# fundamentalvision/BEVFormer

Measured on NVIDIA H100. Metric: BEV queries/sec (bevformer_base 200x200x256, 6 cams) fwd+bwd, higher is better.
Workload: dtype bf16

## Files before the change

### bevformer_b200/_lib.py

```python
from __future__ import annotations

import ctypes
import os
import threading

from . import build as _build

_lock = threading.Lock()
_lib = None

c_void_p, c_int, c_int64 = ctypes.c_void_p, ctypes.c_int, ctypes.c_int64

SIGNATURES = {
    "bevf_version": (c_int, []),
    "bevf_last_error": (ctypes.c_char_p, []),
    "bevf_launch_count": (c_int64, []),
    "bevf_msda_forward": (c_int, [c_void_p, c_int, c_void_p, c_void_p, c_void_p, c_void_p,
                                  c_void_p, c_int] + [c_int] * 7 + [c_void_p]),
    "bevf_msda_backward": (c_int, [c_void_p, c_int, c_void_p, c_void_p, c_void_p, c_void_p,
                                   c_void_p, c_int, c_void_p, c_void_p, c_void_p] + [c_int] * 7
                           + [c_void_p]),
    "bevf_msda_rows_forward": (c_int, [c_void_p, c_int, c_void_p, c_void_p, c_void_p, c_void_p,
                                       c_void_p, c_int, c_void_p] + [c_int] * 7 + [c_void_p]),
    "bevf_msda_rows_backward": (c_int, [c_void_p, c_int, c_void_p, c_void_p, c_void_p, c_void_p,
                                        c_void_p, c_int, c_void_p, c_void_p, c_void_p, c_void_p]
                                + [c_int] * 7 + [c_void_p]),
    "bevf_msda_rows_backward_ordered": (c_int, [c_void_p, c_int, c_void_p, c_void_p, c_void_p, c_void_p,
                                                c_void_p, c_int, c_void_p, c_void_p, c_void_p, c_void_p,
                                                c_void_p] + [c_int] * 7 + [c_void_p]),
    "bevf_msda_set_backward_mode": (c_int, [c_int]),
    "bevf_abs_max": (c_int, [c_void_p, c_int, c_int64, c_void_p, c_void_p]),
    "bevf_msda_rows_backward_f16acc": (c_int, [c_void_p, c_int, c_void_p, c_void_p, c_void_p, c_void_p, c_void_p, c_int,
                                               c_void_p, c_void_p, c_void_p, c_void_p, c_void_p, c_void_p] + [c_int] * 7
                                       + [c_void_p]),
    "bevf_gv16_unscale": (c_int, [c_void_p, c_void_p, c_void_p, c_int64, c_void_p]),
    "bevf_msda_rows_backward_mixed": (c_int, [c_void_p, c_int, c_void_p, c_void_p, c_void_p, c_void_p, c_void_p, c_void_p,
                                              c_int, c_void_p, c_void_p, c_void_p, c_int, c_void_p, c_void_p, c_void_p,
                                              c_void_p] + [c_int] * 7 + [c_void_p]),
    "bevf_msda_rows_backward_mixed_dense": (c_int, [c_void_p, c_int, c_void_p, c_void_p, c_void_p, c_void_p, c_void_p,
                                                    c_void_p, c_int, c_void_p, c_void_p, c_void_p, c_int, c_int,
                                                    c_void_p, c_void_p, c_void_p, c_void_p] + [c_int] * 7 + [c_void_p]),
    "bevf_gv_merge": (c_int, [c_void_p, c_void_p, c_void_p, c_void_p, c_int, c_int, c_int, c_int, c_void_p]),
    "bevf_msda_fx_frac_bits": (c_int, [c_int64, c_int, c_int]),
    "bevf_msda_backward_fx": (c_int, [c_void_p, c_int, c_void_p, c_void_p, c_void_p, c_void_p, c_void_p, c_int,
                                      c_void_p, c_void_p, c_int, c_void_p, c_void_p] + [c_int] * 7 + [c_void_p]),
    "bevf_msda_rows_backward_fx": (c_int, [c_void_p, c_int, c_void_p, c_void_p, c_void_p, c_void_p, c_void_p, c_int,
                                           c_void_p, c_void_p, c_int, c_void_p, c_void_p, c_void_p] + [c_int] * 7
                                   + [c_void_p]),
    "bevf_msda_fx_convert": (c_int, [c_void_p, c_void_p, c_int, c_void_p, c_int, c_int, c_int64, c_void_p]),
    "bevf_msda_rows_backward_dense": (c_int, [c_void_p, c_int, c_void_p, c_void_p, c_void_p, c_void_p, c_void_p,
                                              c_void_p, c_int, c_void_p, c_void_p, c_void_p, c_void_p, c_void_p]
                                      + [c_int] * 7 + [c_void_p]),
    "bevf_msda_set_dense_backward": (c_int, [c_int]),
    "bevf_msda_get_dense_backward": (c_int, []),
    "bevf_msda_dense_plan": (c_int, [c_void_p, c_int, c_int, c_int, c_void_p, c_int, c_void_p]),
    "bevf_sca_plan_workspace_ints": (c_int64, [c_int, c_int]),
    "bevf_sca_plan_build": (c_int, [c_void_p] * 10 + [c_int] * 5 + [c_void_p]),
    "bevf_sca_prep_forward": (c_int, [c_void_p] * 7 + [c_int] * 8 + [c_void_p]),
    "bevf_sca_prep_backward": (c_int, [c_void_p] * 6 + [c_int] * 8 + [c_void_p]),
    "bevf_sca_rows_forward_fused": (c_int, [c_void_p, c_int] + [c_void_p] * 9 + [c_int, c_void_p, c_int, c_void_p]
                                    + [c_int] * 12 + [c_void_p]),
    "bevf_sca_rows_backward_fused": (c_int, [c_void_p, c_int] + [c_void_p] * 7 + [c_int] + [c_void_p] * 5
                                     + [c_int, c_void_p, c_void_p, c_void_p, c_int, c_int] + [c_void_p] * 5
                                     + [c_int] * 12 + [c_void_p]),
    "bevf_sca_prep_backward_multi": (c_int, [c_void_p] * 6 + [c_int] * 8 + [c_void_p]),
    "bevf_tsa_prep_forward": (c_int, [c_void_p] * 5 + [c_int] * 6 + [c_void_p]),
    "bevf_tsa_prep_backward": (c_int, [c_void_p] * 5 + [c_int] * 7 + [c_void_p]),
    "bevf_query_prep_forward": (c_int, [c_void_p] * 5 + [c_int] * 7 + [c_void_p]),
    "bevf_query_prep_backward": (c_int, [c_void_p] * 5 + [c_int] * 8 + [c_void_p]),
    "bevf_refine_points": (c_int, [c_void_p, c_int64, c_void_p, c_void_p, c_void_p, c_int, c_int64, c_void_p]),
    "bevf_layernorm_forward": (c_int, [c_void_p] * 4 + [c_int] + [c_void_p] * 5
                               + [c_int64, c_int, ctypes.c_float, ctypes.c_float, ctypes.c_uint64, c_void_p,
                                  c_int, c_void_p]),
    "bevf_layernorm_backward": (c_int, [c_void_p] * 3 + [c_int] + [c_void_p] * 4 + [c_int64]
                                + [c_void_p] * 4
                                + [c_int64, c_int, ctypes.c_float, ctypes.c_uint64, c_void_p, c_int,
                                   c_void_p]),
    "bevf_layernorm_backward_workspace_bytes": (c_int64, [c_int64, c_int]),
    "bevf_layernorm_backward_det": (c_int, [c_void_p] * 3 + [c_int] + [c_void_p] * 4 + [c_int64]
                                    + [c_void_p] * 5 + [c_int64]
                                    + [c_int64, c_int, ctypes.c_float, ctypes.c_uint64, c_void_p, c_int,
                                       c_void_p]),
    "bevf_sca_combine_forward": (c_int, [c_void_p] * 4 + [c_int] * 6 + [c_void_p]),
    "bevf_sca_combine_backward": (c_int, [c_void_p] * 4 + [c_int] * 5 + [c_void_p]),
    "bevf_linear_forward": (c_int, [c_void_p] * 3 + [c_int] + [c_void_p] * 2
                            + [c_int, c_int64, c_int, c_int, c_int, c_void_p]),
    "bevf_flatten_feats": (c_int, [c_void_p] * 4 + [c_int] * 7 + [c_void_p]),
    "bevf_linear_dgrad": (c_int, [c_void_p] * 3 + [c_int64, c_int, c_int, c_void_p]),
    "bevf_linear_dgrad_acc": (c_int, [c_void_p] * 4 + [c_int64, c_int, c_int, c_void_p]),
    "bevf_linear_wgrad": (c_int, [c_void_p] * 4 + [c_int64, c_int, c_int, c_void_p]),
    "bevf_linear_wgrad_workspace_bytes": (c_int64, [c_int64, c_int, c_int]),
    "bevf_linear_wgrad_out": (c_int, [c_void_p] * 4 + [c_int, c_void_p, c_int64, c_int64, c_int, c_int,
                                                      c_void_p]),
    "bevf_sum_tensors": (c_int, [c_void_p, c_int, c_void_p, c_int64, c_int, c_void_p]),
    "bevf_linear_wgrad_into": (c_int, [c_void_p] * 5 + [c_int64, c_int64, c_int, c_int, c_void_p]),
    "bevf_linear_forward_dt": (c_int, [c_void_p] * 3 + [c_int] + [c_void_p] * 2
                               + [c_int, c_int64, c_int, c_int, c_int, c_int, c_void_p]),
    "bevf_linear_dgrad_dt": (c_int, [c_void_p] * 3 + [c_int64, c_int, c_int, c_int, c_void_p]),
    "bevf_linear_dgrad_acc_dt": (c_int, [c_void_p] * 4 + [c_int64, c_int, c_int, c_int, c_void_p]),
    "bevf_linear_wgrad_dt": (c_int, [c_void_p] * 4 + [c_int64, c_int, c_int, c_int, c_void_p]),
    "bevf_linear_wgrad_out_dt": (c_int, [c_void_p] * 4 + [c_int, c_void_p, c_int64, c_int64, c_int, c_int, c_int,
                                                         c_void_p]),
    "bevf_linear_wgrad_into_dt": (c_int, [c_void_p] * 5 + [c_int64, c_int64, c_int, c_int, c_int, c_void_p]),
    "bevf_colsum": (c_int, [c_void_p, c_void_p, c_int64, c_int, c_int, c_void_p]),
    "bevf_colsum_workspace_bytes": (c_int64, [c_int64, c_int]),
    "bevf_colsum_det": (c_int, [c_void_p, c_void_p, c_void_p, c_int64, c_int64, c_int, c_int, c_void_p]),
    "bevf_dropout_inplace": (c_int, [c_void_p, c_int64, ctypes.c_float, ctypes.c_uint64, c_void_p, c_int,
                                     c_void_p]),
# ... 75 lines not shown
```

### bevformer_b200/csrc/msda.cu

```cuda
#include <cuda_fp16.h>

#include <cstdlib>
#include <cstring>
#include <mutex>
#include <type_traits>

#include "msda_common.cuh"

namespace bevf {

template <typename T, typename TO, bool kFused = false>
__global__ void __launch_bounds__(kThreads)
msda_fwd_d32(const T *__restrict__ value, const int64_t *__restrict__ level_hw,
             const int64_t *__restrict__ level_start, const float *__restrict__ loc,
             const float *__restrict__ attn, TO *__restrict__ out,
             const int *__restrict__ row_map, int S, int M, int Q, int L, int P, int magic,
             int iters, long long rows, const __grid_constant__ ScaFuse fz = ScaFuse{}) {
    constexpr int VEC = Vec<T>::N, LANES = 32 / VEC, G = 32 / LANES;
    static_assert(!kFused || LANES == 4, "the fused prep needs 4 lanes per row (16-bit value rows)");
    constexpr bool kHalf = std::is_same<T, bf16>::value;
    __shared__ __align__(16) float s_fa[kFused ? kThreads / 32 * G : 1][kFuseLP];
    __shared__ LevelTab tab;
    load_level_tab(level_hw, level_start, L, M * 32, tab);

// ... 514 lines not shown
    return 0;
}

template <typename T, typename TO>
static int launch_fwd(const char *who, const void *value, const int64_t *hw, const int64_t *ls,
                      const float *loc, const float *attn, void *out, const int *row_map, int S,
                      int M, int D, int Q, int L, int P, long long rows, cudaStream_t st,
                      const ScaFuse *fz = nullptr) {
    if (D == 32) {
        const unsigned grid = grid_d32(rows, Vec<T>::N);
        if (fz) {
            if constexpr (std::is_same<T, bf16>::value && std::is_same<TO, bf16>::value)
                msda_fwd_d32<T, TO, true><<<grid, kThreads, 0, st>>>((const T *)value, hw, ls, nullptr, nullptr, (TO *)out,
                                                                     row_map, S, M, Q, L, P, (65536 + P - 1) / P, 1,
                                                                     rows, *fz);
            else
                return fail("%s: the fused prep needs bf16 value and output", who);
        } else {
            msda_fwd_d32<T, TO><<<grid, kThreads, 0, st>>>((const T *)value, hw, ls, loc, attn, (TO *)out,
                                                           row_map, S, M, Q, L, P, (65536 + P - 1) / P, 1,
                                                           rows);
        }
    } else if (fz) {
        return fail("%s: the fused prep needs head_dim 32", who);
    } else {
        const unsigned grid = (unsigned)((rows + kThreads / 32 - 1) / (kThreads / 32));
        msda_fwd_generic<T, TO><<<grid, kThreads, 0, st>>>((const T *)value, hw, ls, loc, attn,
                                                           (TO *)out, row_map, S, M, D, Q, L, P, rows);
    }
    return check_launch(who);
}

static std::atomic<int> g_bwd_mode{-1};
static int bwd_split_enabled() {
    int v = g_bwd_mode.load(std::memory_order_relaxed);
    if (v < 0) {
        const char *e = getenv("BEVF_MSDA_BWD");
        v = (e && e[0] == 's') ? 1 : 0;
        g_bwd_mode.store(v, std::memory_order_relaxed);
    }
    return v;
}
static unsigned splat_direct_mask() {
    static long v = -1;
    if (v < 0) {
        const char *e = getenv("BEVF_SPLAT_DIRECT");
        v = e ? strtol(e, nullptr, 0) : 0;
    }
    return (unsigned)v;
}

int dense_coarse_backward(const char *who, const int64_t *hw_dev, const int64_t *ls_dev, const int32_t *hw_host,
                          const float *loc, const float *attn, const void *grad_out, float *grad_value,
                          const int32_t *map_range, int NB, int S, int M, int L, int P, cudaStream_t st,
                          unsigned *handled, HostLevels *host_levels, int first_level, unsigned need_mask,
                          int gv_S, int gv_base, int loc_level0);

static cudaStream_t g_side_stream = nullptr;
constexpr int kSideEvents = 64;
static cudaEvent_t g_side_events[kSideEvents];
static std::atomic<unsigned> g_side_ev_next{0};

template <typename TG, int kM>
static int launch_splat_km(const char *who, const float *loc, const float *attn, const void *go, float *gv,
                           const int *row_map, const int *order, const int64_t *hw, const int64_t *ls,
                           int S, int M, int Q, int L, int P, long long pairs, unsigned level_mask,
                           cudaStream_t st) {
    static bool attr_done = false;
    if (!attr_done) {
        if (cudaFuncSetAttribute(msda_bwd_splat_d32<TG, kM>, cudaFuncAttributeMaxDynamicSharedMemorySize,
                                 (int)splat_smem_bytes(kSplatMaxHeads, sizeof(TG))) != cudaSuccess) {
            cudaGetLastError();
            return fail("%s: cannot reserve shared memory for the splat kernel", who);
        }
        attr_done = true;
    }
    const unsigned grid = (unsigned)((pairs + kSplatG - 1) / kSplatG);
    msda_bwd_splat_d32<TG, kM><<<grid, 32 * M, splat_smem_bytes(M, sizeof(TG)), st>>>(
        loc, attn, (const TG *)go, gv, row_map, order, hw, ls, S, M, Q, L, P, pairs, splat_direct_mask(),
        level_mask);
    return check_launch(who);
}

template <typename TG>
static int launch_splat(const char *who, const float *loc, const float *attn, const void *go, float *gv,
                        const int *row_map, const int *order, const int64_t *hw, const int64_t *ls,
                        int S, int M, int Q, int L, int P, long long pairs, unsigned level_mask,
                        cudaStream_t st) {
    if constexpr (std::is_same<TG, __half>::value) {
        return fail("%s: the splat kernel takes fp32 or bf16 grad_out", who);
    } else {
        if (M == 8)
            return launch_splat_km<TG, 8>(who, loc, attn, go, gv, row_map, order, hw, ls, S, M, Q, L, P, pairs,
                                          level_mask, st);
        return launch_splat_km<TG, 0>(who, loc, attn, go, gv, row_map, order, hw, ls, S, M, Q, L, P, pairs,
                                      level_mask, st);
    }
}

struct MixedGv {
    const unsigned *amax = nullptr;
    __half *gv16 = nullptr;
    unsigned mask = 0;
    int side_start = 0, S_side = 0;
};

struct FxGv {
    const unsigned *bounds = nullptr;
    int frac_bits = 0;
// ... 246 lines not shown
    cudaStream_t s = nullptr;
    if (cudaStreamCreateWithFlags(&s, cudaStreamNonBlocking) != cudaSuccess) {
        cudaGetLastError();
        return fail("%s: cannot create the second stream", who);
    }
    for (int i = 0; i < kSideEvents; ++i) cudaEventCreateWithFlags(&g_side_events[i], cudaEventDisableTiming);
    g_side_stream = s;
    return 0;
}

extern "C" int bevf_msda_set_dense_backward(int mode) {
    if (mode < -1 || mode > 2)
        return fail("%s: mode must be -1 (library default), 0 (off), 1 (same stream) or 2 (second stream)",
                    "bevf_msda_set_dense_backward");
    if (mode == 2)
        if (int e = ensure_side_stream("bevf_msda_set_dense_backward")) return e;
    g_dense_mode.store(mode, std::memory_order_relaxed);
    return 0;
}

extern "C" int bevf_msda_get_dense_backward(void) { return mixed_dense_mode(); }

extern "C" int bevf_msda_rows_backward_dense(const void *value, int value_dtype, const int64_t *level_hw,
                                             const int64_t *level_start, const int32_t *level_hw_host,
                                             const float *loc, const float *attn, const void *grad_out,
                                             int grad_out_dtype, float *grad_value, float *grad_loc,
                                             float *grad_attn, const int32_t *row_map, const int32_t *map_range,
                                             int B, int S, int M, int D, int R, int L, int P, void *stream) {
    const char *who = "bevf_msda_rows_backward_dense";
    if (!row_map && R > 0) return fail("%s: row_map is null", who);
    if (int e = check_dims(who, B, S, M, D, R, L, P)) return e;
    if (R == 0) return 0;
    if (!level_hw_host || !map_range || !level_hw || !level_start || !loc || !attn || !grad_out || !grad_value)
        return fail("%s: null pointer argument", who);
    cudaStream_t st = (cudaStream_t)stream;
    unsigned handled = 0;
    HostLevels hl;
    memset(&hl, 0, sizeof(hl));
    const int mode = dense_setting() < 0 ? 0 : dense_setting();
    cudaEvent_t join = nullptr;
    if (value_dtype == BEVF_DTYPE_F16 || grad_out_dtype == BEVF_DTYPE_F16)
        return fail("%s: fp32 or bf16 only (fp16 runs on bevf_msda_rows_backward)", who);
    if (mode != 0 && D == 32 && grad_out_dtype == BEVF_DTYPE_BF16 && aligned16(loc) && aligned16(attn) &&
        aligned16(grad_out) && aligned16(grad_value)) {
        cudaStream_t ds = st;
        if (mode == 2 && g_side_stream) {
            cudaEvent_t fork = g_side_events[g_side_ev_next.fetch_add(1) % kSideEvents];
            join = g_side_events[g_side_ev_next.fetch_add(1) % kSideEvents];
            cudaEventRecord(fork, st);
            cudaStreamWaitEvent(g_side_stream, fork, 0);
            ds = g_side_stream;
        }
        const int e = dense_coarse_backward(who, level_hw, level_start, level_hw_host, loc, attn, grad_out, grad_value,
                                            map_range, B, S, M, L, P, ds, &handled, &hl, 0, 0u, S, 0, 0);
        if (join) cudaEventRecord(join, g_side_stream);
        if (e) {
            if (join) cudaStreamWaitEvent(st, join, 0);
            return e;
        }
    }
    const int e = msda_backward_impl(who, value, value_dtype, level_hw, level_start, loc, attn, grad_out,
                                     grad_out_dtype, grad_value, grad_loc, grad_attn, row_map, nullptr, B, S, M, D,
                                     R, L, P, stream, handled, &hl);
    if (join) cudaStreamWaitEvent(st, join, 0);
    return e;
}

extern "C" int bevf_msda_rows_backward_f16acc(const void *value, int value_dtype, const int64_t *level_hw,
                                              const int64_t *level_start, const float *loc, const float *attn,
                                              const void *grad_out, int grad_out_dtype, void *grad_value_f16,
                                              const uint32_t *amax_bits, float *grad_loc, float *grad_attn,
                                              const int32_t *row_map, const int32_t *group_order, int B, int S,
                                              int M, int D, int R, int L, int P, void *stream) {
    const char *who = "bevf_msda_rows_backward_f16acc";
    if (!row_map && R > 0) return fail("%s: row_map is null", who);
    if (!grad_value_f16 || !amax_bits) return fail("%s: null pointer argument", who);
    MixedGv mx;
    mx.amax = amax_bits;
    return msda_backward_impl(who, value, value_dtype, level_hw, level_start, loc, attn, grad_out, grad_out_dtype,
                              reinterpret_cast<float *>(grad_value_f16), grad_loc, grad_attn, row_map, group_order, B, S,
                              M, D, R, L, P, stream, 0u, nullptr, true, &mx);
}

static int rows_backward_mixed_impl(const char *who, const void *value, int value_dtype, const int64_t *level_hw,
                                    const int64_t *level_start, const int32_t *level_hw_host, const float *loc,
                                    const float *attn, const void *grad_out, int grad_out_dtype,
                                    void *grad_value_fine_f16, float *grad_value_side, const uint32_t *amax_bits,
                                    int num_f16_levels, int first_dense_level, float *grad_loc, float *grad_attn,
                                    const int32_t *row_map, const int32_t *group_order, const int32_t *map_range,
                                    int B, int S, int M, int D, int R, int L, int P, void *stream,
                                    const ScaFuse *fz = nullptr) {
    if (!row_map && R > 0) return fail("%s: row_map is null", who);
    if (!level_hw_host || !grad_value_fine_f16 || !grad_value_side || !amax_bits)
        return fail("%s: null pointer argument", who);
    if (L <= 1 || L > kMaxLevels || num_f16_levels < 1 || num_f16_levels >= L)
        return fail("%s: num_f16_levels must be in [1, L - 1]", who);
    if (map_range && (first_dense_level < num_f16_levels || first_dense_level >= L))
        return fail("%s: first_dense_level must be in [num_f16_levels, L - 1]", who);
    if (value_dtype != BEVF_DTYPE_BF16 || D != 32) return fail("%s: needs a bf16 value tensor and head_dim 32", who);
    if (!aligned16(grad_value_fine_f16) || !aligned16(grad_value_side))
        return fail("%s: device pointers must be 16-byte aligned", who);
    HostLevels hl;
    memset(&hl, 0, sizeof(hl));
    long long start = 0;
    for (int l = 0; l < L; ++l) {
        const int h = level_hw_host[2 * l], w = level_hw_host[2 * l + 1];
        if (h <= 0 || w <= 0 || h >= 32768 || w >= 32768) return fail("%s: bad host level shape", who);
        hl.h[l] = h; hl.w[l] = w; hl.start[l] = (int)start;
        start += (long long)h * w;
    }
    if (start != S) return fail("%s: host level shapes do not add up to S (%lld vs %lld)", who, start, S);
    MixedGv mx;
    mx.amax = amax_bits;
    mx.gv16 = reinterpret_cast<__half *>(grad_value_fine_f16);
    mx.mask = (1u << num_f16_levels) - 1u;
    mx.side_start = hl.start[num_f16_levels];
    mx.S_side = S - mx.side_start;
    cudaStream_t st = (cudaStream_t)stream;
    unsigned dense_levels = 0;
    cudaEvent_t join = nullptr;
    const int mode = map_range ? mixed_dense_mode() : 0;
    const float *dloc = fz ? reinterpret_cast<const float *>(fz->coarse_loc) : loc;
    const float *dattn = fz ? fz->coarse_attn : attn;
    const int loc_level0 = fz ? fz->coarse_from : 0;
    if (mode != 0 && R > 0 && grad_out_dtype == BEVF_DTYPE_BF16 && aligned16(dloc) && aligned16(dattn) &&
        aligned16(grad_out) && dloc && dattn && loc_level0 <= first_dense_level) {
        cudaStream_t ds = st;
        if (mode == 2 && !g_side_stream) {
            cudaStreamCaptureStatus cs = cudaStreamCaptureStatusActive;
            if (cudaStreamIsCapturing(st, &cs) != cudaSuccess) cudaGetLastError();
            else if (cs == cudaStreamCaptureStatusNone && ensure_side_stream(who) != 0) cudaGetLastError();
        }
        if (mode == 2 && g_side_stream) {
            cudaEvent_t fork = g_side_events[g_side_ev_next.fetch_add(1) % kSideEvents];
            join = g_side_events[g_side_ev_next.fetch_add(1) % kSideEvents];
            cudaEventRecord(fork, st);
            cudaStreamWaitEvent(g_side_stream, fork, 0);
            ds = g_side_stream;
        }
        const unsigned suffix = ((1u << L) - 1u) & ~((1u << first_dense_level) - 1u);
        HostLevels dhl;
        const int e = dense_coarse_backward(who, level_hw, level_start, level_hw_host, dloc, dattn, grad_out,
                                            grad_value_side, map_range, B, S, M, L, P, ds, &dense_levels, &dhl,
                                            first_dense_level, suffix, mx.S_side, mx.side_start, loc_level0);
        if (join) cudaEventRecord(join, g_side_stream);
        if (e) {
            if (join) cudaStreamWaitEvent(st, join, 0);
            return e;
        }
    }
    const int e = msda_backward_impl(who, value, value_dtype, level_hw, level_start, loc, attn, grad_out, grad_out_dtype,
                                     grad_value_side, grad_loc, grad_attn, row_map, group_order, B, S, M, D, R, L, P,
                                     stream, dense_levels, &hl, false, &mx, nullptr, fz);
    if (join) cudaStreamWaitEvent(st, join, 0);
    return e;
}

extern "C" int bevf_msda_rows_backward_mixed(const void *value, int value_dtype, const int64_t *level_hw,
                                             const int64_t *level_start, const int32_t *level_hw_host,
                                             const float *loc, const float *attn, const void *grad_out,
                                             int grad_out_dtype, void *grad_value_fine_f16, float *grad_value_side,
                                             const uint32_t *amax_bits, int num_f16_levels, float *grad_loc,
                                             float *grad_attn, const int32_t *row_map, const int32_t *group_order,
                                             int B, int S, int M, int D, int R, int L, int P, void *stream) {
    return rows_backward_mixed_impl("bevf_msda_rows_backward_mixed", value, value_dtype, level_hw, level_start,
                                    level_hw_host, loc, attn, grad_out, grad_out_dtype, grad_value_fine_f16,
                                    grad_value_side, amax_bits, num_f16_levels, L, grad_loc, grad_attn, row_map,
                                    group_order, nullptr, B, S, M, D, R, L, P, stream);
}

extern "C" int bevf_msda_rows_backward_mixed_dense(const void *value, int value_dtype, const int64_t *level_hw,
                                                   const int64_t *level_start, const int32_t *level_hw_host,
                                                   const float *loc, const float *attn, const void *grad_out,
                                                   int grad_out_dtype, void *grad_value_fine_f16,
                                                   float *grad_value_side, const uint32_t *amax_bits,
                                                   int num_f16_levels, int first_dense_level, float *grad_loc,
                                                   float *grad_attn, const int32_t *row_map, const int32_t *map_range,
                                                   int B, int S, int M, int D, int R, int L, int P, void *stream) {
    const char *who = "bevf_msda_rows_backward_mixed_dense";
    if (!map_range) return fail("%s: null pointer argument", who);
    return rows_backward_mixed_impl(who, value, value_dtype, level_hw, level_start, level_hw_host, loc, attn, grad_out,
                                    grad_out_dtype, grad_value_fine_f16, grad_value_side, amax_bits, num_f16_levels,
                                    first_dense_level, grad_loc, grad_attn, row_map, nullptr, map_range, B, S, M, D, R,
                                    L, P, stream);
}

static int sca_fuse_args(const char *who, const float *raw, const float *ref_cam, const int32_t *pair_q,
                         const int32_t *pair_cam, const int32_t *pair_of, const float *stats, const float *coarse_loc,
                         const float *coarse_attn, int coarse_from, int M, int D, int R, int L, int P, int bs, int Nq,
                         int pairs, int Dz, int ncam, ScaFuse &fz) {
    if (M != kFuseHeads || D != 32 || L * P != kFuseLP)
        return fail("%s: 8 heads, head_dim 32 and num_levels * num_points == 32 only", who);
    if (bs <= 0 || Nq <= 0 || pairs < 0 || (long long)bs * pairs != R || Dz <= 0 || P % Dz != 0 || ncam <= 0 ||
        ncam > 16)
        return fail("%s: bad dimension (rows = bs * pairs, num_points a multiple of the Z anchors, ncam <= 16)", who);
    if (!raw || !ref_cam || !pair_q || !pair_cam || !stats) return fail("%s: null pointer argument", who);
// ... 140 lines not shown
```

### bevformer_b200/csrc/msda_dense.cu

```cuda
#include <cuda.h>

#include <cstdlib>
#include <cstring>
#include <mutex>

#include "msda_common.cuh"

namespace bevf {

constexpr int kDnK = 16;
constexpr int kDnMaxBins = 32;
constexpr int kDnBinLevels = 4;
constexpr int kDnTileBytes = 128 * kDnK * 2;
constexpr int kDnTransposeBytes = 16 * 144;

struct DenseBins {
    int nbins, L;
    int s0[kDnMaxBins], n[kDnMaxBins];
    int nlev[kDnMaxBins];
    int lev[kDnMaxBins][kDnBinLevels];
    HostLevels hl;
};

namespace dn {
// ... 23 lines not shown
__device__ __forceinline__ void fence_async_smem() { asm volatile("fence.proxy.async.shared::cta;" ::: "memory"); }

__device__ __forceinline__ uint64_t desc_sw128(uint32_t addr, uint32_t lbo_bytes) {
    uint64_t d = 0;
    d |= static_cast<uint64_t>((addr & 0x3FFFFu) >> 4);
    d |= static_cast<uint64_t>(lbo_bytes >> 4) << 16;
    d |= static_cast<uint64_t>(1024 >> 4) << 32;
    d |= static_cast<uint64_t>(1) << 62;
    return d;
}
__device__ __forceinline__ void wgmma_m64n32_amn(float (&d)[16], uint64_t da, uint64_t db) {
    asm volatile("wgmma.mma_async.sync.aligned.m64n32k16.f32.bf16.bf16 "
                 "{%0, %1, %2, %3, %4, %5, %6, %7, %8, %9, %10, %11, %12, %13, %14, %15}, %16, %17, 1, 1, 1, 1, 0;\n"
                 : "+f"(d[0]), "+f"(d[1]), "+f"(d[2]), "+f"(d[3]), "+f"(d[4]), "+f"(d[5]), "+f"(d[6]), "+f"(d[7]),
                   "+f"(d[8]), "+f"(d[9]), "+f"(d[10]), "+f"(d[11]), "+f"(d[12]), "+f"(d[13]), "+f"(d[14]), "+f"(d[15])
                 : "l"(da), "l"(db));
}
template <int N> __device__ __forceinline__ void fence_regs(float (&d)[N]) {
#pragma unroll
    for (int i = 0; i < N; ++i) asm volatile("" : "+f"(d[i])::"memory");
}

__device__ __forceinline__ uint32_t slab_off(int row, int k) {
    return ((uint32_t)(row >> 6) << 11) + ((uint32_t)k << 7) + ((((uint32_t)(row >> 3) & 7u) ^ ((uint32_t)k & 7u)) << 4) +
           (((uint32_t)row & 7u) << 1);
}
__device__ __forceinline__ float2 ldg_f2(const float2 *p) {
    float2 v;
    asm volatile("ld.global.nc.v2.f32 {%0, %1}, [%2];" : "=f"(v.x), "=f"(v.y) : "l"(p));
    return v;
}
__device__ __forceinline__ float ldg_f1(const float *p) {
    float v;
    asm volatile("ld.global.nc.f32 %0, [%1];" : "=f"(v) : "l"(p));
    return v;
}
__device__ __forceinline__ uint4 ldg_u4(const uint4 *p) {
    uint4 v;
    asm volatile("ld.global.nc.v4.u32 {%0, %1, %2, %3}, [%4];" : "=r"(v.x), "=r"(v.y), "=r"(v.z), "=r"(v.w) : "l"(p));
    return v;
}
__device__ __forceinline__ unsigned short lds16(uint32_t addr) {
    unsigned short h;
    asm volatile("ld.shared.u16 %0, [%1];" : "=h"(h) : "r"(addr) : "memory");
    return h;
}
__device__ __forceinline__ void sts16(uint32_t addr, unsigned short h) {
    asm volatile("st.shared.u16 [%0], %1;" ::"r"(addr), "h"(h) : "memory");
}
__device__ __forceinline__ unsigned short bf16_add(unsigned short old, float x) {
    const float v = __uint_as_float((uint32_t)old << 16) + x;
    return __bfloat16_as_ushort(__float2bfloat16_rn(v));
}
}

template <int kTiles, int P, int NT>
__global__ void __launch_bounds__(128 * NT + 256, 1)
msda_bwd_dense_tc(const __grid_constant__ DenseBins bins, const int64_t *__restrict__ level_hw,
                  const int64_t *__restrict__ level_start, const float *__restrict__ loc,
                  const float *__restrict__ attn, const bf16 *__restrict__ grad_out,
                  float *__restrict__ grad_value, const int *__restrict__ map_range, int NB, int gv_S, int gv_base,
                  int M, int L, int chunk_rows, int dbg, int loc_level0) {
    static_assert(P == 4 || P == 8, "points per level: 4 or 8");
    static_assert(kTiles == 4, "accumulator tiles per bin: 2 per issuer warpgroup");
    static_assert(NT >= 1 && NT <= 3, "scatter teams");
    constexpr int kThreadsAll = 128 * NT + 256;
    constexpr int kSlabBytes = kTiles * kDnTileBytes;
    constexpr int kMine = kTiles / 2;
    constexpr int kColsPerWarp = 32 / P;
    constexpr int kWarpsPerLevel = kDnK / kColsPerWarp;
    constexpr int kLevelsPerPass = 4 / kWarpsPerLevel;
    constexpr int kMaxPass = kDnBinLevels / kLevelsPerPass;
    extern __shared__ __align__(1024) uint8_t smem_raw[];
    uint8_t *smem = reinterpret_cast<uint8_t *>((reinterpret_cast<uintptr_t>(smem_raw) + 1023) & ~uintptr_t(1023));
    uint8_t *slab = smem;
    uint8_t *gtile = smem + NT * kSlabBytes;
    float *tr = reinterpret_cast<float *>(gtile + NT * 4096);
    uint64_t *bar_full = reinterpret_cast<uint64_t *>(reinterpret_cast<uint8_t *>(tr) + 8 * kDnTransposeBytes);
    uint64_t *bar_empty = bar_full + NT;
    uint32_t *s_dirty = reinterpret_cast<uint32_t *>(bar_empty + NT);
    __shared__ int s_h[kMaxLevels], s_w[kMaxLevels], s_start[kMaxLevels];
    __shared__ int s_bad;

    const int tid = threadIdx.x, lane = tid & 31;
    const int team = tid >> 7, tt = tid & 127, tw = tt >> 5;
    const bool is_team = team < NT;

    if (tid == 0) s_bad = 0;
    __syncthreads();
    if (tid < L) {
        s_h[tid] = (int)level_hw[2 * tid];
        s_w[tid] = (int)level_hw[2 * tid + 1];
        s_start[tid] = (int)level_start[tid];
    }
    if (tid == 64 && !host_levels_match(bins.hl, level_hw, level_start, L)) s_bad = 1;
    if (tid == 32) {
        for (int i = 0; i < NT; ++i) { dn::mbar_init(&bar_full[i], 128); dn::mbar_init(&bar_empty[i], 8); }
        asm volatile("fence.mbarrier_init.release.cluster;" ::: "memory");
        for (int i = 0; i < 2 * NT; ++i) s_dirty[i] = 0;
    }
    {
        uint4 *z = reinterpret_cast<uint4 *>(smem);
        const int n16 = (NT * kSlabBytes + NT * 4096) / 16;
        for (int i = tid; i < n16; i += kThreadsAll) z[i] = make_uint4(0, 0, 0, 0);
    }
    __syncthreads();
    if (s_bad) return;
    dn::fence_async_smem();
    __syncthreads();

    const int per_chunk = M * bins.nbins;
    int total = 0;
    for (int b = 0; b < NB; ++b) {
        const int n = __ldg(map_range + 2 * b + 1) - __ldg(map_range + 2 * b);
        total += ((n + chunk_rows - 1) / chunk_rows) * per_chunk;
    }

    const int k = (tw % kWarpsPerLevel) * kColsPerWarp + lane / P, pt = lane % P, lsub = tw / kWarpsPerLevel;
    const uint32_t my_slab = dn::s32(slab + (is_team ? team : 0) * kSlabBytes) + ((uint32_t)k << 7);
    const uint32_t kx = (uint32_t)k & 7u;
    const uint32_t my_gt = dn::s32(gtile + (is_team ? team : 0) * 4096);
    const bool g_role = is_team && tt < 64;
    const int gk = tt & 15, gc = (tt >> 4) & 3;
    uint32_t nuse = 0;
    uint32_t nfull[NT];
#pragma unroll
    for (int i = 0; i < NT; ++i) nfull[i] = 0;
    float acc[kMine][2][16];
    auto unit_bar = [] { asm volatile("bar.sync 1, %0;" ::"n"(kThreadsAll) : "memory"); };

    auto row_off = [&](int row) -> uint32_t {
        return ((uint32_t)(row >> 6) << 11) + ((((uint32_t)(row >> 3) & 7u) ^ kx) << 4) + (((uint32_t)row & 7u) << 1);
    };

    for (int u = blockIdx.x; u < total; u += gridDim.x) {
        int b = 0, rem = u, ps = 0, pe = 0;
        for (; b < NB; ++b) {
            ps = __ldg(map_range + 2 * b); pe = __ldg(map_range + 2 * b + 1);
            const int cnt = ((pe - ps + chunk_rows - 1) / chunk_rows) * per_chunk;
            if (rem < cnt) break;
            rem -= cnt;
        }
        const int chunk = rem / per_chunk, rem2 = rem - chunk * per_chunk;
        const int m = rem2 / bins.nbins, bin = rem2 - m * bins.nbins;
        const int r_begin = ps + chunk * chunk_rows, r_end = min(pe, r_begin + chunk_rows);
        const int nsteps = (r_end - r_begin + kDnK - 1) / kDnK;
        const int s0 = bins.s0[bin], nb = bins.n[bin];

        if (is_team) {
            const int nlev = bins.nlev[bin];
            int lv[kMaxPass], Hq[kMaxPass], Wq[kMaxPass], lb[kMaxPass];
            bool on[kMaxPass];
            uint32_t rec_a[kMaxPass], rec_b[kMaxPass];
#pragma unroll
            for (int q = 0; q < kMaxPass; ++q) {
                const int slot = q * kLevelsPerPass + lsub;
                on[q] = slot < nlev;
                lv[q] = on[q] ? bins.lev[bin][slot] : 0;
                Hq[q] = s_h[lv[q]]; Wq[q] = s_w[lv[q]]; lb[q] = s_start[lv[q]] - s0;
                rec_a[q] = rec_b[q] = 0;
            }
            struct Smp { float x, y, a; };
            auto load_samples = [&](int step, Smp (&q)[kMaxPass]) {
                const int r = r_begin + step * kDnK + k;
                const bool live = step < nsteps && r < r_end;
#pragma unroll
                for (int i = 0; i < kMaxPass; ++i) {
                    q[i].x = q[i].y = q[i].a = 0.f;
                    if (live && on[i]) {
                        const long long e = (((long long)r * M + m) * (L - loc_level0) + lv[i] - loc_level0) * P + pt;
                        const float2 xy = dn::ldg_f2(reinterpret_cast<const float2 *>(loc) + e);
                        q[i].x = xy.x; q[i].y = xy.y; q[i].a = dn::ldg_f1(attn + e);
                    }
                }
            };
            auto load_gout = [&](int step) -> uint4 {
                const int r = r_begin + step * kDnK + gk;
                if (g_role && step < nsteps && r < r_end)
                    return dn::ldg_u4(reinterpret_cast<const uint4 *>(grad_out + ((long long)r * M + m) * 32 + gc * 8));
                return make_uint4(0, 0, 0, 0);
            };
            auto unscatter = [&]() {
#pragma unroll
                for (int q = 0; q < kMaxPass; ++q) {
                    const uint32_t ra = rec_a[q], rb = rec_b[q];
                    if ((ra | rb) != 0) {
                        if (ra & 0x8000u) dn::sts16(my_slab + ((ra & 0x7fffu) << 1), 0);
                        if (ra & 0x80000000u) dn::sts16(my_slab + (((ra >> 16) & 0x7fffu) << 1), 0);
                        if (rb & 0x8000u) dn::sts16(my_slab + ((rb & 0x7fffu) << 1), 0);
                        if (rb & 0x80000000u) dn::sts16(my_slab + (((rb >> 16) & 0x7fffu) << 1), 0);
                        rec_a[q] = rec_b[q] = 0;
                    }
                }
            };
            auto corner_round = [&](bool act, uint32_t off, float cf, int row, uint32_t &dirty) -> uint32_t {
                const uint32_t key = act ? (my_slab + off) : (0xffffff00u | (uint32_t)lane);
                const unsigned peers = __match_any_sync(0xffffffffu, key);
                float sum = cf;
// ... 120 lines not shown
#pragma unroll
                for (int i = 0; i < kMine; ++i) { dn::fence_regs(acc[i][0]); dn::fence_regs(acc[i][1]); }
                udirty |= mask;
                __syncwarp();
                if (lane == 0) dn::mbar_arrive(&bar_empty[t]);
                if (++t == NT) t = 0;
            }
            unit_bar();
            if (!(dbg & (4 | 1))) {
                float *trw = tr + (iw * 4 + w4) * (kDnTransposeBytes / 4);
                const int sub = lane & 7;
#pragma unroll
                for (int i = 0; i < kMine; ++i) {
                    const int tile = 2 * i + iw;
                    if (!((udirty >> tile) & 1u)) continue;
#pragma unroll
                    for (int h = 0; h < 2; ++h) {
#pragma unroll
                        for (int j = 0; j < 4; ++j)
#pragma unroll
                            for (int hh = 0; hh < 2; ++hh)
                                *reinterpret_cast<float2 *>(trw + (8 * hh + (lane >> 2)) * 36 + 8 * j + 2 * (lane & 3)) =
                                    make_float2(acc[i][h][4 * j + 2 * hh], acc[i][h][4 * j + 2 * hh + 1]);
                        __syncwarp();
#pragma unroll
                        for (int q = 0; q < 4; ++q) {
                            const int rr = 4 * q + (lane >> 3);
                            const int row = tile * 128 + h * 64 + w4 * 16 + rr;
                            const float4 v = *reinterpret_cast<const float4 *>(trw + rr * 36 + sub * 4);
                            const bool nz = ((__float_as_uint(v.x) | __float_as_uint(v.y) | __float_as_uint(v.z) |
                                              __float_as_uint(v.w)) & 0x7fffffffu) != 0u;
                            if (nz && row < nb) {
                                float *gp = grad_value + (((long long)b * gv_S + s0 - gv_base + row) * M + m) * 32 + sub * 4;
                                red_add_v4(gp, v.x, v.y, v.z, v.w);
                            }
                        }
                        __syncwarp();
                    }
                }
            }
            unit_bar();
        }
    }
}

}

namespace bevf {

static long dense_env(const char *name, long dflt) {
    const char *e = getenv(name);
    return e ? strtol(e, nullptr, 0) : dflt;
}

static int plan_dense_bins(const int32_t *hw_host, int L, long max_pix, int cap, DenseBins &bins, long long *total,
                           int first = 0) {
    memset(&bins, 0, sizeof(bins));
    bins.L = L;
    long long start = 0;
    unsigned mask = 0;
    int open = -1;
    for (int l = 0; l < L; ++l) {
        const int h = hw_host[2 * l], w = hw_host[2 * l + 1];
        if (h <= 0 || w <= 0 || h >= 32768 || w >= 32768) return -1;
        const long long n = (long long)h * w;
        bins.hl.h[l] = h; bins.hl.w[l] = w; bins.hl.start[l] = (int)start;
        if (l >= first && n <= max_pix) {
            if (n <= cap && open >= 0 && bins.n[open] + n <= cap && bins.nlev[open] < kDnBinLevels) {
                bins.lev[open][bins.nlev[open]++] = l;
                bins.n[open] += (int)n;
            } else {
                const int parts = (int)((n + cap - 1) / cap);
                if (bins.nbins + parts > kDnMaxBins) return -2;
                long long off = 0;
                for (int i = 0; i < parts; ++i) {
                    const int bi = bins.nbins++;
                    bins.s0[bi] = (int)(start + off);
                    bins.n[bi] = (int)((n - off) < cap ? (n - off) : cap);
                    bins.nlev[bi] = 1;
                    bins.lev[bi][0] = l;
                    off += bins.n[bi];
                }
                open = bins.nbins - 1;
            }
            mask |= 1u << l;
        } else {
            open = -1;
        }
        start += n;
    }
    *total = start;
    return (int)mask;
}

int dense_coarse_backward(const char *who, const int64_t *hw_dev, const int64_t *ls_dev, const int32_t *hw_host,
                          const float *loc, const float *attn, const void *grad_out, float *grad_value,
                          const int32_t *map_range, int NB, int S, int M, int L, int P, cudaStream_t st,
                          unsigned *handled, HostLevels *host_levels, int first_level, unsigned need_mask,
                          int gv_S, int gv_base, int loc_level0) {
    *handled = 0;
    static const long max_pix = dense_env("BEVF_DENSE_MAXPIX", 8192);
    static const long tiles = dense_env("BEVF_DENSE_TILES", 4);
    static const long chunk = dense_env("BEVF_DENSE_CHUNK", 512);
    if ((P != 4 && P != 8) || L > kMaxLevels || NB <= 0 || max_pix <= 0) return 0;
    if (tiles != 4) return fail("%s: BEVF_DENSE_TILES must be 4", who);
    if (chunk < kDnK || chunk % kDnK) return fail("%s: BEVF_DENSE_CHUNK must be a positive multiple of 16", who);
    const int cap = (int)tiles * 128;
    DenseBins bins;
    long long start = 0;
    const int pm = plan_dense_bins(hw_host, L, max_pix, cap, bins, &start, first_level);
    if (pm == -1) return fail("%s: bad host level shape", who);
    if (pm == -2) return 0;
    const unsigned mask = (unsigned)pm;
    if (start != S) return fail("%s: host level shapes do not add up to S (%lld vs %lld)", who, start, S);
    if (mask == 0 || (need_mask != 0 && mask != need_mask)) return 0;
    static int sms = 0;
    if (sms == 0) {
        int dev = 0;
        cudaGetDevice(&dev);
        cudaDeviceGetAttribute(&sms, cudaDevAttrMultiProcessorCount, dev);
    }
    static const long teams_env = dense_env("BEVF_DENSE_TEAMS", 0);
    const int teams = teams_env > 0 ? (int)teams_env : 3;
    const size_t smem = 1024 + (size_t)teams * ((size_t)tiles * kDnTileBytes + 4096) + 8 * kDnTransposeBytes + 256;
    static const long dbg = dense_env("BEVF_DENSE_DEBUG", 0);
    auto launch = [&](auto kern) -> int {
        static const void *configured[16];
        static int nconfigured = 0;
        static std::mutex mu;
        {
            std::lock_guard<std::mutex> lock(mu);
            bool seen = false;
            for (int i = 0; i < nconfigured; ++i) seen = seen || configured[i] == (const void *)kern;
            if (!seen) {
                if (cudaFuncSetAttribute(kern, cudaFuncAttributeMaxDynamicSharedMemorySize, (int)smem) != cudaSuccess) {
                    cudaGetLastError();
                    return fail("%s: cannot reserve shared memory for the dense backward", who);
                }
                if (nconfigured < 16) configured[nconfigured++] = (const void *)kern;
            }
        }
        kern<<<(unsigned)sms, 128 * teams + 256, smem, st>>>(bins, hw_dev, ls_dev, loc, attn, (const bf16 *)grad_out,
                                                           grad_value, map_range, NB, gv_S, gv_base, M, L, (int)chunk,
                                                           (int)dbg, loc_level0);
        return check_launch(who);
    };
    int e;
    if (teams < 1 || teams > 3) return fail("%s: BEVF_DENSE_TEAMS must be 1, 2 or 3", who);
    if (teams == 3) e = (P == 8) ? launch(msda_bwd_dense_tc<4, 8, 3>) : launch(msda_bwd_dense_tc<4, 4, 3>);
    else if (teams == 2) e = (P == 8) ? launch(msda_bwd_dense_tc<4, 8, 2>) : launch(msda_bwd_dense_tc<4, 4, 2>);
    else e = (P == 8) ? launch(msda_bwd_dense_tc<4, 8, 1>) : launch(msda_bwd_dense_tc<4, 4, 1>);
    if (e) return e;
    *handled = mask;
    *host_levels = bins.hl;
    return 0;
}

}

extern "C" int bevf_msda_dense_plan(const int32_t *level_hw_host, int L, int max_pix, int tiles, int32_t *bins_out,
                                    int bins_cap, uint32_t *level_mask) {
    using namespace bevf;
    const char *who = "bevf_msda_dense_plan";
    if (!level_hw_host || !bins_out || !level_mask || L <= 0 || L > kMaxLevels || (tiles != 4 && tiles != 8 && tiles != 16))
        return -fail("%s: bad argument", who);
    DenseBins bins;
    long long total = 0;
    const int pm = plan_dense_bins(level_hw_host, L, max_pix, tiles * 128, bins, &total);
    if (pm == -1) return -fail("%s: bad host level shape", who);
    if (pm == -2) { *level_mask = 0; return 0; }
    if (bins.nbins > bins_cap) return -fail("%s: output too small", who);
    for (int i = 0; i < bins.nbins; ++i) {
        int32_t *o = bins_out + i * (3 + kDnBinLevels);
        o[0] = bins.s0[i]; o[1] = bins.n[i]; o[2] = bins.nlev[i];
        for (int j = 0; j < kDnBinLevels; ++j) o[3 + j] = j < bins.nlev[i] ? bins.lev[i][j] : -1;
    }
    *level_mask = (unsigned)pm;
    return bins.nbins;
}
```

### include/bevformer_b200.h

```cpp
#ifndef BEVFORMER_B200_H_
#define BEVFORMER_B200_H_

#include <stdint.h>

#ifdef __cplusplus
extern "C" {
#endif

#define BEVF_ABI_VERSION 3

#if defined(__GNUC__)
#define BEVF_API __attribute__((visibility("default")))
#else
#define BEVF_API
#endif

enum bevf_dtype { BEVF_DTYPE_F32 = 0, BEVF_DTYPE_BF16 = 1, BEVF_DTYPE_F16 = 2 };

BEVF_API int bevf_version(void);

BEVF_API const char *bevf_last_error(void);

BEVF_API int64_t bevf_launch_count(void);

// ... 26 lines not shown
                                             float *grad_attn, const int32_t *row_map,
                                             const int32_t *group_order, int B, int S, int M, int D,
                                             int R, int L, int P, void *stream);

BEVF_API int bevf_abs_max(const void *x, int dtype, int64_t n, uint32_t *amax_bits, void *stream);
BEVF_API int bevf_msda_rows_backward_f16acc(const void *value, int value_dtype, const int64_t *level_hw,
                                            const int64_t *level_start, const float *loc, const float *attn,
                                            const void *grad_out, int grad_out_dtype, void *grad_value_f16,
                                            const uint32_t *amax_bits, float *grad_loc, float *grad_attn,
                                            const int32_t *row_map, const int32_t *group_order, int B, int S,
                                            int M, int D, int R, int L, int P, void *stream);
BEVF_API int bevf_gv16_unscale(const void *gv16, const uint32_t *amax_bits, void *out_bf16, int64_t n, void *stream);
BEVF_API int bevf_msda_rows_backward_mixed(const void *value, int value_dtype, const int64_t *level_hw,
                                           const int64_t *level_start, const int32_t *level_hw_host,
                                           const float *loc, const float *attn, const void *grad_out,
                                           int grad_out_dtype, void *grad_value_fine_f16, float *grad_value_side,
                                           const uint32_t *amax_bits, int num_f16_levels, float *grad_loc,
                                           float *grad_attn, const int32_t *row_map, const int32_t *group_order,
                                           int B, int S, int M, int D, int R, int L, int P, void *stream);
BEVF_API int bevf_msda_rows_backward_mixed_dense(const void *value, int value_dtype, const int64_t *level_hw,
                                                 const int64_t *level_start, const int32_t *level_hw_host,
                                                 const float *loc, const float *attn, const void *grad_out,
                                                 int grad_out_dtype, void *grad_value_fine_f16, float *grad_value_side,
                                                 const uint32_t *amax_bits, int num_f16_levels, int first_dense_level,
                                                 float *grad_loc, float *grad_attn, const int32_t *row_map,
                                                 const int32_t *map_range,
                                                 int B, int S, int M, int D, int R, int L, int P, void *stream);
BEVF_API int bevf_gv_merge(const void *fine_f16, const float *side_f32, const uint32_t *amax_bits, void *out_bf16,
                           int B, int S, int S_fine, int row_elems, void *stream);

BEVF_API int bevf_msda_fx_frac_bits(int64_t rows_per_map, int L, int P);
BEVF_API int bevf_msda_backward_fx(const void *value, int value_dtype, const int64_t *level_hw,
                                   const int64_t *level_start, const float *loc, const float *attn,
                                   const void *grad_out, int grad_out_dtype, int64_t *grad_value_fx, uint32_t *bounds,
                                   int frac_bits, float *grad_loc, float *grad_attn, int B, int S, int M, int D, int Q,
                                   int L, int P, void *stream);
BEVF_API int bevf_msda_rows_backward_fx(const void *value, int value_dtype, const int64_t *level_hw,
                                        const int64_t *level_start, const float *loc, const float *attn,
                                        const void *grad_out, int grad_out_dtype, int64_t *grad_value_fx,
                                        uint32_t *bounds, int frac_bits, float *grad_loc, float *grad_attn,
                                        const int32_t *row_map, int B, int S, int M, int D, int R, int L, int P,
                                        void *stream);
BEVF_API int bevf_msda_fx_convert(const int64_t *grad_value_fx, const uint32_t *bounds, int frac_bits, void *out,
                                  int out_dtype, int accumulate, int64_t n, void *stream);

BEVF_API int bevf_msda_rows_backward_dense(const void *value, int value_dtype, const int64_t *level_hw,
                                           const int64_t *level_start, const int32_t *level_hw_host,
                                           const float *loc, const float *attn, const void *grad_out,
                                           int grad_out_dtype, float *grad_value, float *grad_loc,
                                           float *grad_attn, const int32_t *row_map, const int32_t *map_range,
                                           int B, int S, int M, int D, int R, int L, int P, void *stream);
BEVF_API int bevf_msda_set_dense_backward(int mode);
BEVF_API int bevf_msda_get_dense_backward(void);
BEVF_API int bevf_msda_dense_plan(const int32_t *level_hw_host, int L, int max_pix, int tiles, int32_t *bins_out,
                                  int bins_cap, uint32_t *level_mask);

BEVF_API int bevf_msda_set_backward_mode(int mode);


BEVF_API int64_t bevf_sca_plan_workspace_ints(int ncam, int Nq);
BEVF_API int bevf_sca_plan_build(const unsigned char *bev_mask, const int32_t *qorder, int32_t *pair_q,
                                 int32_t *pair_cam, int32_t *pair_of, int32_t *row_map, float *inv_count,
                                 int32_t *map_range, int32_t *counters, int32_t *workspace, int B, int ncam,
                                 int Nq, int D, int capacity, void *stream);

BEVF_API int bevf_sca_prep_forward(const float *raw, const float *ref_cam, const int32_t *pair_q,
                                   const int32_t *pair_cam, const int64_t *level_hw, float *loc,
                                   float *attn, int B, int Nq, int R, int M, int L, int P, int D,
                                   int ncam, void *stream);

BEVF_API int bevf_sca_prep_backward(const float *raw, const float *grad_loc, const float *grad_attn,
                                    const int32_t *pair_of, const int64_t *level_hw, void *d_raw,
                                    int out_dtype, int B, int Nq, int R, int M, int L, int P, int ncam,
                                    void *stream);

BEVF_API int bevf_sca_rows_forward_fused(const void *value, int value_dtype, const int64_t *level_hw,
                                         const int64_t *level_start, const float *raw, const float *ref_cam,
                                         const int32_t *pair_q, const int32_t *pair_cam, float *stats,
                                         float *coarse_loc, float *coarse_attn, int coarse_from, void *out,
                                         int out_dtype, const int32_t *row_map, int B, int S, int M, int D, int R,
                                         int L, int P, int bs, int Nq, int pairs, int Dz, int ncam, void *stream);

BEVF_API int bevf_sca_rows_backward_fused(const void *value, int value_dtype, const int64_t *level_hw,
                                          const int64_t *level_start, const int32_t *level_hw_host, const float *raw,
                                          const float *stats, const float *coarse_loc, const float *coarse_attn,
                                          int coarse_from, const float *ref_cam, const int32_t *pair_q,
                                          const int32_t *pair_cam, const int32_t *pair_of, const void *grad_out,
                                          int grad_out_dtype, void *grad_value_fine_f16, float *grad_value_side,
                                          const uint32_t *amax_bits, int num_f16_levels, int first_dense_level,
                                          float *grad_loc, float *grad_attn, void *d_raw, const int32_t *row_map,
                                          const int32_t *map_range, int B, int S, int M, int D, int R, int L, int P,
                                          int bs, int Nq, int pairs, int Dz, int ncam, void *stream);

BEVF_API int bevf_sca_prep_backward_multi(const float *raw, const float *grad_loc, const float *grad_attn,
                                          const int32_t *pair_of, const int64_t *level_hw, void *d_raw,
                                          int out_dtype, int B, int Nq, int R, int M, int L, int P, int ncam,
                                          void *stream);

BEVF_API int bevf_tsa_prep_forward(const float *raw, const float *ref2d, const int64_t *level_hw,
                                   float *loc, float *attn, int B, int Nq, int M, int L, int P,
                                   int interleave, void *stream);

BEVF_API int bevf_tsa_prep_backward(const float *raw, const float *grad_loc, const float *grad_attn,
                                    const int64_t *level_hw, void *d_raw, int out_dtype, int B, int Nq,
                                    int M, int L, int P, int interleave, void *stream);

BEVF_API int bevf_query_prep_forward(const float *raw, const float *ref2d, const int64_t *level_hw,
                                     float *loc, float *attn, int B, int Nq, int M, int L, int P, int F,
// ... 150 lines not shown
```

Baseline: 1.752 million.

## Limit dense backward grid on side stream, prioritize it, reorder work units

When the dense coarse-level backward runs concurrently on the side stream, its grid now uses only a fraction of the SMs (one fifth by default), bounded by the number of work units, and the kernel is launched at the highest stream priority. Work units are reordered so full row chunks are scheduled first and partial tail chunks follow, largest first. Together these aim to let the dense kernel overlap with the splat backward on the main stream instead of occupying every SM. The smaller grid may lengthen the dense kernel's critical path, and each unit now recomputes its chunk mapping with O(NB^2) loops over map_range.

```diff
diff --git a/bevformer_b200/_lib.py b/bevformer_b200/_lib.py
--- a/bevformer_b200/_lib.py
+++ b/bevformer_b200/_lib.py
@@ -54,6 +54,9 @@
     "bevf_msda_set_dense_backward": (c_int, [c_int]),
     "bevf_msda_get_dense_backward": (c_int, []),
     "bevf_msda_dense_plan": (c_int, [c_void_p, c_int, c_int, c_int, c_void_p, c_int, c_void_p]),
+    "bevf_msda_set_dense_sms": (c_int, [c_int]),
+    "bevf_msda_get_dense_sms": (c_int, []),
+    "bevf_msda_dense_schedule": (c_int, [c_void_p] + [c_int] * 6 + [c_void_p, c_int, c_void_p]),
     "bevf_sca_plan_workspace_ints": (c_int64, [c_int, c_int]),
     "bevf_sca_plan_build": (c_int, [c_void_p] * 10 + [c_int] * 5 + [c_void_p]),
     "bevf_sca_prep_forward": (c_int, [c_void_p] * 7 + [c_int] * 8 + [c_void_p]),
diff --git a/bevformer_b200/csrc/msda.cu b/bevformer_b200/csrc/msda.cu
--- a/bevformer_b200/csrc/msda.cu
+++ b/bevformer_b200/csrc/msda.cu
@@ -590,9 +590,9 @@
 
 int dense_coarse_backward(const char *who, const int64_t *hw_dev, const int64_t *ls_dev, const int32_t *hw_host,
                           const float *loc, const float *attn, const void *grad_out, float *grad_value,
-                          const int32_t *map_range, int NB, int S, int M, int L, int P, cudaStream_t st,
-                          unsigned *handled, HostLevels *host_levels, int first_level, unsigned need_mask,
-                          int gv_S, int gv_base, int loc_level0);
+                          const int32_t *map_range, int NB, int S, int M, int L, int P, long long R, bool concurrent,
+                          cudaStream_t st, unsigned *handled, HostLevels *host_levels, int first_level,
+                          unsigned need_mask, int gv_S, int gv_base, int loc_level0);
 
 static cudaStream_t g_side_stream = nullptr;
 constexpr int kSideEvents = 64;
@@ -945,7 +945,8 @@
             ds = g_side_stream;
         }
         const int e = dense_coarse_backward(who, level_hw, level_start, level_hw_host, loc, attn, grad_out, grad_value,
-                                            map_range, B, S, M, L, P, ds, &handled, &hl, 0, 0u, S, 0, 0);
+                                            map_range, B, S, M, L, P, R, ds != st, ds, &handled, &hl, 0, 0u, S, 0,
+                                            0);
         if (join) cudaEventRecord(join, g_side_stream);
         if (e) {
             if (join) cudaStreamWaitEvent(st, join, 0);
@@ -1034,7 +1035,8 @@
         const unsigned suffix = ((1u << L) - 1u) & ~((1u << first_dense_level) - 1u);
         HostLevels dhl;
         const int e = dense_coarse_backward(who, level_hw, level_start, level_hw_host, dloc, dattn, grad_out,
-                                            grad_value_side, map_range, B, S, M, L, P, ds, &dense_levels, &dhl,
+                                            grad_value_side, map_range, B, S, M, L, P, R, ds != st, ds,
+                                            &dense_levels, &dhl,
                                             first_dense_level, suffix, mx.S_side, mx.side_start, loc_level0);
         if (join) cudaEventRecord(join, g_side_stream);
         if (e) {
diff --git a/bevformer_b200/csrc/msda_dense.cu b/bevformer_b200/csrc/msda_dense.cu
--- a/bevformer_b200/csrc/msda_dense.cu
+++ b/bevformer_b200/csrc/msda_dense.cu
@@ -99,6 +99,49 @@
     const float v = __uint_as_float((uint32_t)old << 16) + x;
     return __bfloat16_as_ushort(__float2bfloat16_rn(v));
 }
+}
+
+__host__ __device__ __forceinline__ int dn_ld(const int *p) {
+#ifdef __CUDA_ARCH__
+    return __ldg(p);
+#else
+    return *p;
+#endif
+}
+
+__host__ __device__ inline int dense_units_total(const int *map_range, int NB, int chunk_rows, int per_chunk) {
+    int total = 0;
+    for (int b = 0; b < NB; ++b) {
+        const int n = dn_ld(map_range + 2 * b + 1) - dn_ld(map_range + 2 * b);
+        total += ((n + chunk_rows - 1) / chunk_rows) * per_chunk;
+    }
+    return total;
+}
+__host__ __device__ inline void dense_unit(int u, const int *map_range, int NB, int chunk_rows, int per_chunk, int &b,
+                                           int &r_begin, int &r_end, int &rem) {
+    int c = u / per_chunk;
+    rem = u - c * per_chunk;
+    int full = 0;
+    for (int i = 0; i < NB; ++i) full += (dn_ld(map_range + 2 * i + 1) - dn_ld(map_range + 2 * i)) / chunk_rows;
+    b = 0; r_begin = r_end = 0;
+    if (c < full) {
+        for (int i = 0; i < NB; ++i) {
+            const int ps = dn_ld(map_range + 2 * i), f = (dn_ld(map_range + 2 * i + 1) - ps) / chunk_rows;
+            if (c < f) { b = i; r_begin = ps + c * chunk_rows; r_end = r_begin + chunk_rows; return; }
+            c -= f;
+        }
+    }
+    const int j = c - full;
+    for (int i = 0; i < NB; ++i) {
+        const int ps = dn_ld(map_range + 2 * i), pe = dn_ld(map_range + 2 * i + 1), t = (pe - ps) % chunk_rows;
+        if (t == 0) continue;
+        int rank = 0;
+        for (int i2 = 0; i2 < NB; ++i2) {
+            const int t2 = (dn_ld(map_range + 2 * i2 + 1) - dn_ld(map_range + 2 * i2)) % chunk_rows;
+            rank += (t2 > t || (t2 == t && i2 < i)) ? 1 : 0;
+        }
+        if (rank == j) { b = i; r_begin = pe - t; r_end = pe; return; }
+    }
 }
 
 template <int kTiles, int P, int NT>
@@ -157,11 +200,7 @@
     __syncthreads();
 
     const int per_chunk = M * bins.nbins;
-    int total = 0;
-    for (int b = 0; b < NB; ++b) {
-        const int n = __ldg(map_range + 2 * b + 1) - __ldg(map_range + 2 * b);
-        total += ((n + chunk_rows - 1) / chunk_rows) * per_chunk;
-    }
+    const int total = dense_units_total(map_range, NB, chunk_rows, per_chunk);
 
     const int k = (tw % kWarpsPerLevel) * kColsPerWarp + lane / P, pt = lane % P, lsub = tw / kWarpsPerLevel;
     const uint32_t my_slab = dn::s32(slab + (is_team ? team : 0) * kSlabBytes) + ((uint32_t)k << 7);
@@ -181,16 +220,9 @@
     };
 
     for (int u = blockIdx.x; u < total; u += gridDim.x) {
-        int b = 0, rem = u, ps = 0, pe = 0;
-        for (; b < NB; ++b) {
-            ps = __ldg(map_range + 2 * b); pe = __ldg(map_range + 2 * b + 1);
-            const int cnt = ((pe - ps + chunk_rows - 1) / chunk_rows) * per_chunk;
-            if (rem < cnt) break;
-            rem -= cnt;
-        }
-        const int chunk = rem / per_chunk, rem2 = rem - chunk * per_chunk;
+        int b, r_begin, r_end, rem2;
+        dense_unit(u, map_range, NB, chunk_rows, per_chunk, b, r_begin, r_end, rem2);
         const int m = rem2 / bins.nbins, bin = rem2 - m * bins.nbins;
-        const int r_begin = ps + chunk * chunk_rows, r_end = min(pe, r_begin + chunk_rows);
         const int nsteps = (r_end - r_begin + kDnK - 1) / kDnK;
         const int s0 = bins.s0[bin], nb = bins.n[bin];
 
@@ -417,6 +449,23 @@
     const char *e = getenv(name);
     return e ? strtol(e, nullptr, 0) : dflt;
 }
+static long dense_chunk_rows() {
+    static const long chunk = dense_env("BEVF_DENSE_CHUNK", 512);
+    return chunk;
+}
+
+static std::atomic<int> g_dense_sms{-1};
+constexpr int kDenseSmsNum = 1, kDenseSmsDen = 5;
+static int dense_grid(int setting, bool concurrent, int sms, long long unit_bound) {
+    int k = sms;
+    if (setting > 0) k = setting < sms ? setting : sms;
+    else if (concurrent) k = sms * kDenseSmsNum / kDenseSmsDen;
+    if (unit_bound < k) k = (int)unit_bound;
+    return k > 1 ? k : 1;
+}
+static long long dense_unit_bound(long long R, int NB, int M, int nbins, long chunk) {
+    return (R / chunk + NB) * (long long)M * nbins;
+}
 
 static int plan_dense_bins(const int32_t *hw_host, int L, long max_pix, int cap, DenseBins &bins, long long *total,
                            int first = 0) {
@@ -460,13 +509,13 @@
 
 int dense_coarse_backward(const char *who, const int64_t *hw_dev, const int64_t *ls_dev, const int32_t *hw_host,
                           const float *loc, const float *attn, const void *grad_out, float *grad_value,
-                          const int32_t *map_range, int NB, int S, int M, int L, int P, cudaStream_t st,
-                          unsigned *handled, HostLevels *host_levels, int first_level, unsigned need_mask,
-                          int gv_S, int gv_base, int loc_level0) {
+                          const int32_t *map_range, int NB, int S, int M, int L, int P, long long R, bool concurrent,
+                          cudaStream_t st, unsigned *handled, HostLevels *host_levels, int first_level,
+                          unsigned need_mask, int gv_S, int gv_base, int loc_level0) {
     *handled = 0;
     static const long max_pix = dense_env("BEVF_DENSE_MAXPIX", 8192);
     static const long tiles = dense_env("BEVF_DENSE_TILES", 4);
-    static const long chunk = dense_env("BEVF_DENSE_CHUNK", 512);
+    const long chunk = dense_chunk_rows();
     if ((P != 4 && P != 8) || L > kMaxLevels || NB <= 0 || max_pix <= 0) return 0;
     if (tiles != 4) return fail("%s: BEVF_DENSE_TILES must be 4", who);
     if (chunk < kDnK || chunk % kDnK) return fail("%s: BEVF_DENSE_CHUNK must be a positive multiple of 16", who);
@@ -479,12 +528,15 @@
     const unsigned mask = (unsigned)pm;
     if (start != S) return fail("%s: host level shapes do not add up to S (%lld vs %lld)", who, start, S);
     if (mask == 0 || (need_mask != 0 && mask != need_mask)) return 0;
-    static int sms = 0;
-    if (sms == 0) {
-        int dev = 0;
-        cudaGetDevice(&dev);
-        cudaDeviceGetAttribute(&sms, cudaDevAttrMultiProcessorCount, dev);
-    }
+    const int ctas = dense_grid(g_dense_sms.load(std::memory_order_relaxed), concurrent, device_sms(),
+                                dense_unit_bound(R, NB, M, bins.nbins, chunk));
+    static int prio = 0;
+    static std::once_flag prio_once;
+    std::call_once(prio_once, [] {
+        int least = 0, greatest = 0;
+        if (cudaDeviceGetStreamPriorityRange(&least, &greatest) == cudaSuccess) prio = greatest;
+        else cudaGetLastError();
+    });
     static const long teams_env = dense_env("BEVF_DENSE_TEAMS", 0);
     const int teams = teams_env > 0 ? (int)teams_env : 3;
     const size_t smem = 1024 + (size_t)teams * ((size_t)tiles * kDnTileBytes + 4096) + 8 * kDnTransposeBytes + 256;
@@ -505,9 +557,22 @@
                 if (nconfigured < 16) configured[nconfigured++] = (const void *)kern;
             }
         }
-        kern<<<(unsigned)sms, 128 * teams + 256, smem, st>>>(bins, hw_dev, ls_dev, loc, attn, (const bf16 *)grad_out,
-                                                           grad_value, map_range, NB, gv_S, gv_base, M, L, (int)chunk,
-                                                           (int)dbg, loc_level0);
+        cudaLaunchConfig_t cfg = {};
+        cfg.gridDim = dim3((unsigned)ctas);
+        cfg.blockDim = dim3(128 * teams + 256);
+        cfg.dynamicSmemBytes = smem;
+        cfg.stream = st;
+        cudaLaunchAttribute attr[1];
+        attr[0].id = cudaLaunchAttributePriority;
+        attr[0].val.priority = prio;
+        cfg.attrs = attr;
+        cfg.numAttrs = concurrent ? 1 : 0;
+        if (cudaLaunchKernelEx(&cfg, kern, bins, hw_dev, ls_dev, loc, attn, (const bf16 *)grad_out, grad_value,
+                               (const int *)map_range, NB, gv_S, gv_base, M, L, (int)chunk, (int)dbg,
+                               loc_level0) != cudaSuccess) {
+            cudaGetLastError();
+            return fail("%s: dense backward launch failed", who);
+        }
         return check_launch(who);
     };
     int e;
@@ -543,3 +608,35 @@
     *level_mask = (unsigned)pm;
     return bins.nbins;
 }
+
+extern "C" int bevf_msda_set_dense_sms(int sms) {
+    if (sms < -1 || sms == 0)
+        return bevf::fail("%s: sms must be -1 (library default) or a positive SM count", "bevf_msda_set_dense_sms");
+    bevf::g_dense_sms.store(sms, std::memory_order_relaxed);
+    return 0;
+}
+
+extern "C" int bevf_msda_get_dense_sms(void) {
+    return bevf::dense_grid(bevf::g_dense_sms.load(std::memory_order_relaxed), true, bevf::device_sms(), 1ll << 40);
+}
+
+extern "C" int bevf_msda_dense_schedule(const int32_t *map_range_host, int NB, int R, int M, int nbins, int sms,
+                                        int concurrent, int32_t *units_out, int units_cap, int32_t *ctas) {
+    using namespace bevf;
+    const char *who = "bevf_msda_dense_schedule";
+    if (!map_range_host || !ctas || NB <= 0 || R < 0 || M <= 0 || nbins <= 0 || nbins > kDnMaxBins || sms <= 0)
+        return -fail("%s: bad argument", who);
+    const long chunk = dense_chunk_rows();
+    const int per_chunk = M * nbins;
+    const int total = dense_units_total(map_range_host, NB, (int)chunk, per_chunk);
+    if (units_out && total > units_cap) return -fail("%s: output too small", who);
+    for (int u = 0; units_out && u < total; ++u) {
+        int b, r0, r1, rem;
+        dense_unit(u, map_range_host, NB, (int)chunk, per_chunk, b, r0, r1, rem);
+        int32_t *o = units_out + 5 * u;
+        o[0] = b; o[1] = r0; o[2] = r1; o[3] = rem / nbins; o[4] = rem % nbins;
+    }
+    *ctas = dense_grid(g_dense_sms.load(std::memory_order_relaxed), concurrent != 0, sms,
+                       dense_unit_bound(R, NB, M, nbins, chunk));
+    return total;
+}
diff --git a/include/bevformer_b200.h b/include/bevformer_b200.h
--- a/include/bevformer_b200.h
+++ b/include/bevformer_b200.h
@@ -102,8 +102,12 @@
                                            int B, int S, int M, int D, int R, int L, int P, void *stream);
 BEVF_API int bevf_msda_set_dense_backward(int mode);
 BEVF_API int bevf_msda_get_dense_backward(void);
+BEVF_API int bevf_msda_set_dense_sms(int sms);
+BEVF_API int bevf_msda_get_dense_sms(void);
 BEVF_API int bevf_msda_dense_plan(const int32_t *level_hw_host, int L, int max_pix, int tiles, int32_t *bins_out,
                                   int bins_cap, uint32_t *level_mask);
+BEVF_API int bevf_msda_dense_schedule(const int32_t *map_range_host, int NB, int R, int M, int nbins, int sms,
+                                      int concurrent, int32_t *units_out, int units_cap, int32_t *ctas);
 
 BEVF_API int bevf_msda_set_backward_mode(int mode);
 
```

Result: faster. 1.802 million (median of 6 runs) (+2.9%).
